# JettHuang/jet-pbrt

Measured on AMD Instinct MI355X. Metric: Msamples/sec (whole node) + per-pixel L2 vs CPU ref, cornell_box 1024spp, higher is better.
Workload: dtype f32

## Files before the change

### jet-pbrt_amd/__init__.py

```python
import ctypes as C
import os

PKG_DIR = os.path.dirname(os.path.abspath(__file__))
REPO_DIR = os.path.dirname(PKG_DIR)
HIP_LIB_PATH = os.environ.get("JETPBRT_AMD_LIB") or os.path.join(PKG_DIR, "csrc", "libjetpbrt_amd.so")
HOST_LIB_PATH = os.path.join(PKG_DIR, "host", "libjetpbrt_host.so")
CLI_PATH = os.path.join(PKG_DIR, "host", "jetpbrt")

JP_MAT_PARAM_STRIDE = 16
JP_SAMPLER_STOCK_MT19937, JP_SAMPLER_COUNTER, JP_SAMPLER_DEBUG = 0, 1, 2
JP_OK = 0

_fp = C.POINTER(C.c_float)
_ip = C.POINTER(C.c_int32)


class JpCamera(C.Structure):
    _fields_ = [("pos", C.c_float * 3), ("front", C.c_float * 3), ("right", C.c_float * 3), ("up", C.c_float * 3),
                ("res_x", C.c_float), ("res_y", C.c_float)]


class JpScene(C.Structure):
    _fields_ = [
        ("camera", JpCamera),
# ... 1060 lines not shown
        return i

    def set_normal_maps(self, maps):
        self._check(self.lib.jp_set_normal_maps(self.h, None if maps is None else C.byref(maps)))

    def normal_map_info(self):
        i = JpNormalMapInfo()
        i.struct_bytes = C.sizeof(JpNormalMapInfo)
        self._check(self.lib.jp_get_normal_map_info(self.h, C.byref(i)))
        return i

    def set_texture_sampling(self, sampling):
        self._check(self.lib.jp_set_texture_sampling(self.h, None if sampling is None else C.byref(sampling)))

    def texture_sampling_info(self):
        i = JpTexSamplingInfo()
        i.struct_bytes = C.sizeof(JpTexSamplingInfo)
        self._check(self.lib.jp_get_texture_sampling_info(self.h, C.byref(i)))
        return i

    def shading_normal(self, origin, direction, tmin, tmax):
        import numpy as np
        n = origin.shape[0]
        o = np.ascontiguousarray(origin, np.float32); d = np.ascontiguousarray(direction, np.float32)
        t0 = np.ascontiguousarray(tmin, np.float32); t1 = np.ascontiguousarray(tmax, np.float32)
        prim = np.zeros(n, np.int32); ng = np.zeros((n, 3), np.float32); ns = np.zeros((n, 3), np.float32)
        p = lambda a: a.ctypes.data_as(C.c_void_p)
        self._check(self.lib.jp_shading_normal(self.h, n, p(o), p(d), p(t0), p(t1), p(prim), p(ng), p(ns)))
        return prim, ng, ns

    def synchronize(self):
        self._check(self.lib.jp_synchronize(self.h))

    def set_profiling(self, on):
        self._check(self.lib.jp_set_profiling(self.h, 1 if on else 0))

    def counters(self):
        c = JpCounters()
        self._check(self.lib.jp_get_counters(self.h, C.byref(c)))
        return c

    def build_info(self):
        b = JpBuildInfo()
        self._check(self.lib.jp_get_build_info(self.h, C.byref(b)))
        return b

    def shadow_kernel(self):
        fn = self.lib.jp_dbg_shadow_kernel
        fn.argtypes = [C.c_void_p, C.POINTER(C.c_int)]; fn.restype = C.c_int
        which = C.c_int(-1)
        self._check(fn(self.h, C.byref(which)))
        return ("refill", "generic", "flat", "pair")[which.value]

    def read_table(self, which):
        return _read_table(lambda out, cap, n: self.lib.jp_read_scene_table(self.h, _table_index(which), out, cap, n))

    def tree_info(self):
        i = JpTreeInfo()
        i.struct_bytes = C.sizeof(JpTreeInfo)
        self._check(self.lib.jp_get_tree_info(self.h, C.byref(i)))
        return i

    def trace(self, origin, direction, tmin, tmax):
        import numpy as np
        n = origin.shape[0]
        o = np.ascontiguousarray(origin, np.float32); d = np.ascontiguousarray(direction, np.float32)
        t0 = np.ascontiguousarray(tmin, np.float32); t1 = np.ascontiguousarray(tmax, np.float32)
        hit = np.zeros(n, np.int32); t = np.zeros(n, np.float32); prim = np.zeros(n, np.int32); nrm = np.zeros((n, 3), np.float32)
        p = lambda a: a.ctypes.data_as(C.c_void_p)
        self._check(self.lib.jp_trace(self.h, n, p(o), p(d), p(t0), p(t1), p(hit), p(t), p(prim), p(nrm)))
        return hit, t, prim, nrm

    def occluded(self, origin, direction, tmin, tmax):
        import numpy as np
        n = origin.shape[0]
        o = np.ascontiguousarray(origin, np.float32); d = np.ascontiguousarray(direction, np.float32)
        t0 = np.ascontiguousarray(tmin, np.float32); t1 = np.ascontiguousarray(tmax, np.float32)
        occ = np.zeros(n, np.int32); walk = C.c_int32(-1)
        p = lambda a: a.ctypes.data_as(C.c_void_p)
        self._check(self.lib.jp_occluded(self.h, n, p(o), p(d), p(t0), p(t1), p(occ), C.byref(walk)))
        return occ, int(walk.value)

    def bsdf(self, desc, normal, wo, wi, u):
        import numpy as np
        n = normal.shape[0]
        a = [np.ascontiguousarray(x, np.float32) for x in (normal, wo, wi, u)]
        out = dict(f=np.zeros((n, 3), np.float32), pdf=np.zeros(n, np.float32), sf=np.zeros((n, 3), np.float32), swi=np.zeros((n, 3), np.float32),
                   spdf=np.zeros(n, np.float32), sflags=np.zeros(n, np.int32))
        p = lambda x: x.ctypes.data_as(C.c_void_p)
        self._check(self.lib.jp_bsdf(self.h, C.byref(desc), n, p(a[0]), p(a[1]), p(a[2]), p(a[3]), p(out["f"]), p(out["pdf"]), p(out["sf"]), p(out["swi"]), p(out["spdf"]), p(out["sflags"])))
        return out

    def close(self):
        if self.h:
            self.lib.jp_destroy_context(self.h)
            self.h = C.c_void_p()

    def __del__(self):
        try:
            self.close()
        except Exception:
            pass


from . import scenes
from . import distributed
# ... 1 lines not shown
```

### jet-pbrt_amd/csrc/jp_device.h

```cpp
#pragma once
#include <hip/hip_runtime.h>
#include <stdint.h>
#include "jetpbrt_amd.h"
#include "jp_counter_rng.h"

#define JP_BLOCK 256
#define JP_STACK_DEPTH 32

namespace jp
{
struct V3 { float x, y, z; };
__device__ __forceinline__ V3 mk(float x, float y, float z) { V3 v; v.x = x; v.y = y; v.z = z; return v; }
__device__ __forceinline__ V3 operator+(V3 a, V3 b) { return mk(a.x + b.x, a.y + b.y, a.z + b.z); }
__device__ __forceinline__ V3 operator-(V3 a, V3 b) { return mk(a.x - b.x, a.y - b.y, a.z - b.z); }
__device__ __forceinline__ V3 operator-(V3 a) { return mk(-a.x, -a.y, -a.z); }
__device__ __forceinline__ V3 operator*(V3 a, float s) { return mk(a.x * s, a.y * s, a.z * s); }
__device__ __forceinline__ V3 operator*(float s, V3 a) { return mk(a.x * s, a.y * s, a.z * s); }
__device__ __forceinline__ V3 operator/(V3 a, float s) { return mk(a.x / s, a.y / s, a.z / s); }
__device__ __forceinline__ V3 cmul(V3 a, V3 b) { return mk(a.x * b.x, a.y * b.y, a.z * b.z); }
__device__ __forceinline__ V3 cdiv(V3 a, V3 b) { return mk(a.x / b.x, a.y / b.y, a.z / b.z); }
__device__ __forceinline__ V3 splat(float v) { return mk(v, v, v); }
__device__ __forceinline__ V3 csqrt(V3 a) { return mk(sqrtf(a.x), sqrtf(a.y), sqrtf(a.z)); }
__device__ __forceinline__ float dot(V3 a, V3 b) { return a.x * b.x + a.y * b.y + a.z * b.z; }
__device__ __forceinline__ float len2(V3 a) { return a.x * a.x + a.y * a.y + a.z * a.z; }
// ... 334 lines not shown
		#pragma unroll
		for (int u = 0; u < 4; u++) JP_FLAT_BOX(i0 + u)
	}
	for (; i0 < n_flat; i0++) JP_FLAT_BOX(i0)
	#undef JP_FLAT_BOX
	#undef JP_FLAT_BOX_RAY
	mA = maskA; mB = maskB;
}

template <int kS, typename PrimPtr>
__device__ __forceinline__ void flat_prims_pair(unsigned int mA, unsigned int mB, PrimPtr prims, V3 o, V3 dA, V3 dB, float tmin, float tmaxA, float tmaxB, bool& hitA, bool& hitB)
{
	bool hA = false, hB = false;
	unsigned int todo = mA | mB;
	while (todo)
	{
		const int p = __ffs((int)todo) - 1;
		const unsigned int bit = todo & (0u - todo);
		todo &= todo - 1;
		const float4 g0 = prims[kS * p + 0], g1 = prims[kS * p + 1], g2 = prims[kS * p + 2], g3 = prims[kS * p + 3];
		const V3 n = xyz(g3);
		const V3 oa = xyz(g0) - o;
		const float noa = dot(n, oa);
		const float distA = noa / dot(n, dA), distB = noa / dot(n, dB);
		const bool passA = (mA & bit) && (distA > tmin) && (distA < tmaxA);
		const bool passB = (mB & bit) && (distB > tmin) && (distB < tmaxB);
		if (passA || passB)
		{
			const V3 ob = xyz(g1) - o, oc = xyz(g2) - o;
			const V3 v0 = cross(oc, ob), v1 = cross(ob, oa);
			const float v0A = dot(v0, dA), v1A = dot(v1, dA), v0B = dot(v0, dB), v1B = dot(v1, dB);
			bool inA, inB;
			if (__float_as_int(g3.w) == JP_SHAPE_TRIANGLE)
			{
				const V3 v2 = cross(oa, oc);
				const float v2A = dot(v2, dA), v2B = dot(v2, dB);
				inA = ((v0A < 0) && (v1A < 0) && (v2A < 0)) || ((v0A >= 0) && (v1A >= 0) && (v2A >= 0));
				inB = ((v0B < 0) && (v1B < 0) && (v2B < 0)) || ((v0B >= 0) && (v1B >= 0) && (v2B >= 0));
			}
			else
			{
				const V3 od = mk(g0.w, g1.w, g2.w) - o;
				const V3 v2 = cross(oa, od), v3 = cross(od, oc);
				const float v2A = dot(v2, dA), v3A = dot(v3, dA), v2B = dot(v2, dB), v3B = dot(v3, dB);
				inA = ((v0A < 0) && (v1A < 0) && (v2A < 0) && (v3A < 0)) || ((v0A >= 0) && (v1A >= 0) && (v2A >= 0) && (v3A >= 0));
				inB = ((v0B < 0) && (v1B < 0) && (v2B < 0) && (v3B < 0)) || ((v0B >= 0) && (v1B >= 0) && (v2B >= 0) && (v3B >= 0));
			}
			if (passA && inA) { hA = true; mA = 0; }
			if (passB && inB) { hB = true; mB = 0; }
			todo &= mA | mB;
		}
	}
	hitA = hA; hitB = hB;
}

template <bool kAnyHit, typename PrimPtr>
__device__ __forceinline__ int traverse_wide(const uint4* __restrict__ wide, PrimPtr prims, V3 o, V3 d, float tmin, float& tmax, unsigned int* stack)
{
	const float ix = 1.0f / d.x, iy = 1.0f / d.y, iz = 1.0f / d.z;
	const unsigned int octinv = 7u - ((d.x < 0 ? 1u : 0u) | (d.y < 0 ? 2u : 0u) | (d.z < 0 ? 4u : 0u));
	unsigned int ngx = 0, ngy = 0x80000000u;
	int hit = -1, sp = 0;
	for (;;)
	{
		unsigned int tgx = 0, tgy = 0;
		if (ngy > 0x00ffffffu)
		{
			const unsigned int bit = 31u - (unsigned int)__clz((int)ngy);
			ngy &= ~(1u << bit);
			if (ngy > 0x00ffffffu) { stack[(2 * sp) * JP_BLOCK] = ngx; stack[(2 * sp + 1) * JP_BLOCK] = ngy; sp++; }
			const unsigned int slot = (bit - 24u) ^ octinv;
			const unsigned int rel = (unsigned int)__popc(ngy & 0xffu & ~(0xffffffffu << slot));
			const unsigned int idx = ngx + rel;
			const uint4 q0 = wide[5 * idx + 0], q1 = wide[5 * idx + 1], q2 = wide[5 * idx + 2], q3 = wide[5 * idx + 3], q4 = wide[5 * idx + 4];
			const float sx = __uint_as_float(((q0.w & 0xffu) ) << 23), sy = __uint_as_float(((q0.w >> 8) & 0xffu) << 23), sz = __uint_as_float(((q0.w >> 16) & 0xffu) << 23);
			const float px = __uint_as_float(q0.x) - o.x, py = __uint_as_float(q0.y) - o.y, pz = __uint_as_float(q0.z) - o.z;
			unsigned int hm = 0;
			#pragma unroll
			for (int i = 0; i < 8; i++)
			{
				const int sh = 8 * (i & 3);
				const unsigned int m = ((i < 4 ? q1.z : q1.w) >> sh) & 0xffu;
				const float lx = (float)(((i < 4 ? q2.x : q2.y) >> sh) & 0xffu), ly = (float)(((i < 4 ? q2.z : q2.w) >> sh) & 0xffu), lz = (float)(((i < 4 ? q3.x : q3.y) >> sh) & 0xffu);
				const float hx = (float)(((i < 4 ? q3.z : q3.w) >> sh) & 0xffu), hy = (float)(((i < 4 ? q4.x : q4.y) >> sh) & 0xffu), hz = (float)(((i < 4 ? q4.z : q4.w) >> sh) & 0xffu);
				const float x0 = fmaf(lx, sx, px) * ix, x1 = fmaf(hx, sx, px) * ix;
				const float y0 = fmaf(ly, sy, py) * iy, y1 = fmaf(hy, sy, py) * iy;
				const float z0 = fmaf(lz, sz, pz) * iz, z1 = fmaf(hz, sz, pz) * iz;
				const float tn = fmaxf(fmaxf(fminf(x0, x1), fminf(y0, y1)), fmaxf(fminf(z0, z1), tmin));
				const float tf = fminf(fminf(fmaxf(x0, x1), fmaxf(y0, y1)), fminf(fmaxf(z0, z1), tmax));
				if (m != 0u && tn <= tf * 1.000002f)
				{
					const bool inner = (m & 0x18u) == 0x18u;
					const unsigned int bits = inner ? 1u : (m >> 5), at = inner ? 24u + ((m & 7u) ^ octinv) : (m & 31u);
					hm |= bits << at;
				}
			}
			ngx = q1.x; ngy = (hm & 0xff000000u) | (q0.w >> 24);
			tgx = q1.y; tgy = hm & 0x00ffffffu;
		}
		while (tgy)
		{
			const int j = __ffs((int)tgy) - 1;
			tgy &= tgy - 1;
			if (prim_hit<4>(prims, (int)tgx + j, o, d, tmin, tmax)) { hit = (int)tgx + j; if (kAnyHit) return hit; }
		}
		if (ngy <= 0x00ffffffu)
// ... 287 lines not shown
```

### jet-pbrt_amd/csrc/jp_kernels.hip

```cpp
#include "jp_common.h"
#include "jp_tex.h"
#include "jp_normals.h"
#include "jp_normal_map.h"
#include "jp_env.h"
#include "jp_mis.h"
#include "jp_lens.h"
#include "jp_xbsdf.h"
#include "jp_film.h"

#include <cstdio>
#include <cstring>
#include <string>
#include <vector>
#include <algorithm>
#include <cmath>
#include <mutex>
#include <thread>
#include <tuple>
#include <functional>
#include <type_traits>
#include "jp_devmem.h"
#include "jp_lbvh.h"
#include "jp_ploc.h"

// ... 113 lines not shown

template <> struct SceneAccess<3>
{
	const float4* prims; unsigned int* stack;
	__device__ __forceinline__ SceneAccess(const SceneView& sc, int) : prims(sc.prims), stack((unsigned int*)s_dyn + threadIdx.x) {}
	template <bool kAnyHit> __device__ __forceinline__ int trace(const SceneView& sc, V3 o, V3 d, float tmin, float& tmax) const
	{ return traverse_wide<kAnyHit>(sc.wide, prims, o, d, tmin, tmax, stack); }
};

template <> struct SceneAccess<4>
{
	WalkStack stack;
	__device__ __forceinline__ SceneAccess(const SceneView&, int depth) { stack.lds = (int*)s_dyn + threadIdx.x; stack.spill = nullptr; stack.cap = depth - 1; stack.stride = 0; }
	template <bool kAnyHit> __device__ __forceinline__ int trace(const SceneView& sc, V3 o, V3 d, float tmin, float& tmax) const
	{ return walk_ray<4, kAnyHit>(sc, o, d, tmin, tmax, stack); }
};

template <> struct SceneAccess<6>
{
	WalkStack stack;
	__device__ __forceinline__ SceneAccess(const SceneView&, int depth) { stack.lds = (int*)s_dyn + threadIdx.x; stack.spill = nullptr; stack.cap = depth - 1; stack.stride = 0; }
	template <bool kAnyHit> __device__ __forceinline__ int trace(const SceneView& sc, V3 o, V3 d, float tmin, float& tmax) const
	{ return walk_ray<6, kAnyHit>(sc, o, d, tmin, tmax, stack); }
};

template <> struct SceneAccess<5>
{
	const float4 *nodes, *prims; int* stack;
	__device__ __forceinline__ SceneAccess(const SceneView& sc, int) : nodes(sc.nodes), prims(sc.prims), stack((int*)s_dyn + threadIdx.x) {}
	template <bool kAnyHit> __device__ __forceinline__ int trace(const SceneView&, V3 o, V3 d, float tmin, float& tmax) const
	{ return traverse_ref<kAnyHit>(nodes, prims, o, d, tmin, tmax, stack); }
};

template <int kMode, typename F = FeatAll>
__global__ void __launch_bounds__(JP_BLOCK) k_extend(SceneView sc, Queues q, int cur, int depth, DevCounters* cnt)
{
	SceneAccess<kMode, F> acc(sc, depth);
	const unsigned int b = blockIdx.x, n = q.blk_q[cur][b], rbase = b * q.R;
	if (b == 0 && threadIdx.x == 0) { cnt->closest += cnt->n_queue[cur]; cnt->n_queue[cur ^ 1] = 0; cnt->n_shadow = 0; }
	unsigned int h = 0;
	float4 ro = make_float4(0, 0, 0, 0), rd = make_float4(0, 0, 1, 0);
	if (threadIdx.x < n) { ro = q.ray_o[cur][rbase + threadIdx.x]; rd = q.ray_d[cur][rbase + threadIdx.x]; }
	for (unsigned int j = threadIdx.x; j < n; j += JP_BLOCK)
	{
		const unsigned int i = rbase + j;
		const float4 co = ro, cd = rd;
		if (j + JP_BLOCK < n) { ro = q.ray_o[cur][i + JP_BLOCK]; rd = q.ray_d[cur][i + JP_BLOCK]; }
		float tmax = JP_INF;
		int hit;
		if constexpr (kMode == 2) hit = acc.trace_unbounded(sc, xyz(co), xyz(cd), 0.001f, tmax);
		else hit = acc.template trace<false>(sc, xyz(co), xyz(cd), 0.001f, tmax);
		q.hit[i] = make_float2(tmax, __int_as_float(hit));
		h += hit >= 0 ? 1u : 0u;
	}
	for (int off = 32; off > 0; off >>= 1) h += __shfl_down(h, off);
	if ((threadIdx.x & 63) == 0 && h) atomicAdd(&cnt->closest_hit, (unsigned long long)h);
}

#ifndef JP_SHADE_TILE
#define JP_SHADE_TILE 8192
#endif
template <bool kSmooth> struct SmoothVars { };
template <> struct SmoothVars<true> { float4 next, rec; V3 Ns; bool on, guard; };
template <bool kSmooth> __device__ __forceinline__ V3 shade_n(const SmoothVars<kSmooth>& sm, V3 N) { if constexpr (kSmooth) return sm.Ns; else return N; }
template <bool kSmooth> __device__ __forceinline__ bool shade_refuses(const SmoothVars<kSmooth>& sm, V3 w, V3 wo, V3 Ng)
{
	if constexpr (kSmooth) return sm.guard && dot(w, Ng) * dot(wo, Ng) <= 0.f; else return false;
}
template <bool kTab, bool kPrims, bool kStage, bool kSort, bool kTex, bool kPick, bool kEnv, bool kMis, typename F = FeatAll, bool kOne = false, bool kSmooth = false>
__device__ __forceinline__ void shade_body(SceneView sc, Queues q, RenderConst rc, int cur, DevCounters* cnt, const TexView& tv, const PickView& pv, const EnvView& ev, const MisView& mv, const NormView& nv = NormView())
{
	static_assert(kPick || !kMis, "k_shade: the light strategy's pdf needs the light table");
	static_assert(kTab || !kPrims, "k_shade: primitive records in LDS only together with the tables");
	static_assert(kPick || !kEnv, "k_shade: the map light is an entry of the light table");
	static_assert(!kSmooth || !kPrims, "k_shade: a shading normal has no entry in the frame table");
	constexpr int kWaves = JP_BLOCK / 64, kMaxSeg = (JP_SHADE_TILE / JP_BLOCK) * kWaves;
	static_assert(JP_SHADE_TILE % JP_BLOCK == 0 && JP_SHADE_TILE <= 65536, "k_shade: tile positions are 16-bit");
	__shared__ unsigned short s_idx[kSort ? JP_SHADE_TILE : 1];
	static_assert(!kOne || (kSort && kPrims && !F::delta && !F::other_lights && !kTex && !kPick && !kMis), "k_shade: the one-sweep partition is the lean sorted instance's");
	__shared__ unsigned char s_key[kSort && !kOne ? JP_SHADE_TILE : 1];
	__shared__ unsigned int s_cnt[kSort && !kOne ? JP_SHADE_CLASSES * kMaxSeg : 1];
	__shared__ unsigned int s_two;
	__shared__ unsigned int s_wsum[kWaves];
	__shared__ unsigned int s_ctr[3];
	const unsigned int lane = threadIdx.x & 63u;
	const int n_tab_l = kPick ? 0 : 2 * sc.n_lights;
	const int n_tab = n_tab_l + 4 * sc.n_mats + (sc.n_mats + 3) / 4, n_tab_all = n_tab + (kPrims ? 8 * sc.n_prims : 0);
	float4* s_lights = s_dyn;
	float4* s_mats = s_lights + n_tab_l;
	int* s_mtype = (int*)(s_mats + 4 * sc.n_mats);
	float4* s_prims = s_dyn + n_tab;
	int4* s_meta = (int4*)(s_prims + 4 * sc.n_prims);
	const float4* s_frames = s_prims + 5 * sc.n_prims;
	float4* s_stage = s_dyn + n_tab_all + threadIdx.x;
	const unsigned int b = blockIdx.x, n = q.blk_q[cur][b];
	const int nxt = cur ^ 1;
#ifdef JP_SHADE_TIMING
	unsigned long long t_acc[10] = { 0, 0, 0, 0, 0, 0, 0, 0, 0, 0 }, t_last = __builtin_amdgcn_s_memtime();
#endif
	if (kTab)
	{
		for (int i = threadIdx.x; i < n_tab_all; i += 2 * JP_BLOCK)
		{
			const bool two = i + JP_BLOCK < n_tab_all;
			const float4 a = sc.shade_tab[i], c2 = two ? sc.shade_tab[i + JP_BLOCK] : a;
			s_dyn[i] = a; if (two) s_dyn[i + JP_BLOCK] = c2;
// ... 974 lines not shown
		s.wi = to_world(fr, s.wi);
		feval[3 * i] = f.x; feval[3 * i + 1] = f.y; feval[3 * i + 2] = f.z; pdfeval[i] = pe;
		sf[3 * i] = s.f.x; sf[3 * i + 1] = s.f.y; sf[3 * i + 2] = s.f.z;
		swi[3 * i] = s.wi.x; swi[3 * i + 1] = s.wi.y; swi[3 * i + 2] = s.wi.z;
		spdf[i] = s.pdf; sflags[i] = s.flags;
	}
}

template <int kMode>
__global__ void __launch_bounds__(JP_BLOCK) k_trace(SceneView sc, int depth, int n, const float* o, const float* d, const float* tmin, const float* tmax_in,
                                                    int* hit, float* t, int* prim, float* nrm)
{
	SceneAccess<kMode> acc(sc, depth);
	for (int i = blockIdx.x * JP_BLOCK + threadIdx.x; i < n; i += gridDim.x * JP_BLOCK)
	{
		const V3 ro = mk(o[3 * i], o[3 * i + 1], o[3 * i + 2]), rd = mk(d[3 * i], d[3 * i + 1], d[3 * i + 2]);
		float tmax = tmax_in[i];
		const int h = acc.template trace<false>(sc, ro, rd, tmin[i], tmax);
		hit[i] = h >= 0; t[i] = tmax; prim[i] = h >= 0 ? sc.meta[h].x : -1;
		V3 N = mk(0, 0, 0);
		if (h >= 0)
		{
			const float4 g3 = sc.prims[4 * h + 3]; const int type = __float_as_int(g3.w);
			const V3 p = ro + tmax * rd;
			if (type == JP_SHAPE_TRIANGLE) N = xyz(g3);
			else if (type == JP_SHAPE_RECTANGLE) N = dot(xyz(g3), rd) <= 0 ? xyz(g3) : -xyz(g3);
			else if (type == JP_SHAPE_DISK) N = xyz(sc.prims[4 * h + 1]);
			else N = normalize(p - xyz(sc.prims[4 * h]));
		}
		nrm[3 * i] = N.x; nrm[3 * i + 1] = N.y; nrm[3 * i + 2] = N.z;
	}
}

__global__ void __launch_bounds__(JP_BLOCK) k_trace_flat(SceneView sc, int depth, int n, const float* o, const float* d, const float* tmin, const float* tmax_in,
                                                         int* hit, float* t, int* prim, float* nrm)
{
	SceneAccess<2, FeatFlat> acc(sc, depth);
	for (int i = blockIdx.x * JP_BLOCK + threadIdx.x; i < n; i += gridDim.x * JP_BLOCK)
	{
		const V3 ro = mk(o[3 * i], o[3 * i + 1], o[3 * i + 2]), rd = mk(d[3 * i], d[3 * i + 1], d[3 * i + 2]);
		float tmax = tmax_in[i];
		const int h = acc.template trace<false>(sc, ro, rd, tmin[i], tmax);
		hit[i] = h >= 0; t[i] = tmax; prim[i] = h >= 0 ? sc.meta[h].x : -1;
		V3 N = mk(0, 0, 0);
		if (h >= 0)
		{
			const float4 g3 = sc.prims[4 * h + 3];
			N = (__float_as_int(g3.w) == JP_SHAPE_TRIANGLE || dot(xyz(g3), rd) <= 0) ? xyz(g3) : -xyz(g3);
		}
		nrm[3 * i] = N.x; nrm[3 * i + 1] = N.y; nrm[3 * i + 2] = N.z;
	}
}

template <int kMode, typename F = FeatAll>
__global__ void __launch_bounds__(JP_BLOCK) k_occluded(SceneView sc, int depth, int n, const float* o, const float* d, const float* tmin, const float* tmax_in, int* occluded)
{
	SceneAccess<kMode, F> acc(sc, depth);
	for (int i = blockIdx.x * JP_BLOCK + threadIdx.x; i < n; i += gridDim.x * JP_BLOCK)
	{
		const V3 ro = mk(o[3 * i], o[3 * i + 1], o[3 * i + 2]), rd = mk(d[3 * i], d[3 * i + 1], d[3 * i + 2]);
		float tmax = tmax_in[i];
		occluded[i] = acc.template trace<true>(sc, ro, rd, tmin[i], tmax) >= 0;
	}
}

__global__ void __launch_bounds__(JP_BLOCK, 8) k_texel(SceneView sc, Queues q, int cur, TexView tv)
{
	const unsigned int b = blockIdx.x, n = q.blk_q[cur][b], rbase = b * q.R;
	for (unsigned int j = threadIdx.x; j < n; j += JP_BLOCK)
	{
		const unsigned int i = rbase + j;
		const float2 h = q.hit[i];
		const int pi = __float_as_int(h.y);
		unsigned int w = 0u;
		if (pi >= 0)
		{
			const int4 meta = sc.meta[pi];
			const int t = meta.y >= 0 ? tv.mat_tex[meta.y] : -1;
			if (t >= 0)
			{
				const float4 ro = q.ray_o[cur][i], rd = q.ray_d[cur][i];
				const V3 p = xyz(ro) + h.x * xyz(rd);
				w = tex_sample(tv, t, tex_uv(sc.prims, tv, pi, meta.x, p), p);
			}
		}
		tv.side[i] = w;
	}
}

template <bool kTab, bool kPrims, bool kStage, bool kSort>
__global__ void __launch_bounds__(JP_BLOCK) k_shade_tex(SceneView sc, Queues q, RenderConst rc, int cur, DevCounters* cnt, TexView tv)
{
	const PickView pv = {}; const EnvView ev = {}; const MisView mv = {};
	shade_body<kTab, kPrims, kStage, kSort, true, false, false, false>(sc, q, rc, cur, cnt, tv, pv, ev, mv);
}

template <int kMode>
__global__ void __launch_bounds__(JP_BLOCK) k_surface(SceneView sc, TexView tv, int depth, int n, const float* o, const float* d, const float* tmin, const float* tmax_in,
                                                      int* prim, float* uv, float* albedo, SampView sm)
{
	SceneAccess<kMode> acc(sc, depth);
	for (int i = blockIdx.x * JP_BLOCK + threadIdx.x; i < n; i += gridDim.x * JP_BLOCK)
	{
		const V3 ro = mk(o[3 * i], o[3 * i + 1], o[3 * i + 2]), rd = mk(d[3 * i], d[3 * i + 1], d[3 * i + 2]);
		float tmax = tmax_in[i];
		const int h = acc.template trace<false>(sc, ro, rd, tmin[i], tmax);
// ... 46 lines not shown
```

### jet-pbrt_amd/csrc/jp_render.h

```cpp
#pragma once
namespace
{
enum { CLS_EXTEND = 0, CLS_SHADE = 1, CLS_SHADOW = 2, CLS_OTHER = 3, CLS_PATH = 4, CLS_NORMAL = 5, CLS_NMAP = 6, CLS_TEXEL = 7 };

int lens_plan_of(const JpContext* c, JpLensPlan& lp)
{
	std::memset(&lp, 0, sizeof(lp));
	if (!c->lens_on) return JP_OK;
	if (jp_lens_make_plan(&c->plan.sv.cam, &c->lens, &lp) != 0) return fail(JP_ERR_INVALID_ARGUMENT, "jp_set_lens: the uploaded camera's right / up vectors have no finite positive length");
	return JP_OK;
}

void free_queues(JpContext* c) { c->qb = QueueBufs(); c->cap = 0; c->planes_alloc = 0; c->blk_alloc = 0; }

int ensure_queues(JpContext* c, unsigned int cap, int planes, unsigned int nblocks)
{
	if (c->cap >= cap && c->planes_alloc >= planes && c->blk_alloc >= nblocks) return JP_OK;
	cap = std::max(cap, c->cap); planes = std::max(planes, c->planes_alloc); nblocks = std::max(nblocks, c->blk_alloc);
	free_queues(c);
	auto alloc = [](DevBuf& b, auto*& p, size_t bytes) { return reserve(b, p, bytes) == hipSuccess; };
	Queues& q = c->q; QueueBufs& qb = c->qb; bool ok = true;
	for (int b = 0; b < 2 && ok; b++) ok = alloc(qb.ray_o[b], q.ray_o[b], (size_t)cap * 16) && alloc(qb.ray_d[b], q.ray_d[b], (size_t)cap * 16) && alloc(qb.beta[b], q.beta[b], (size_t)cap * 16)
	                                       && alloc(qb.blk_q[b], q.blk_q[b], (size_t)nblocks * 4);
	ok = ok && alloc(qb.hit, q.hit, (size_t)cap * 8) && alloc(qb.lacc, q.lacc, (size_t)cap * 16) && alloc(qb.sh_o, q.sh_o, (size_t)cap * 16)
// ... 32 lines not shown
	{
		if (!c->profiling) return;
		if (c->evused + 2 > c->evpool.size()) { size_t old = c->evpool.size(); c->evpool.resize(old + 64); for (size_t i = old; i < c->evpool.size(); i++) hipEventCreate(&c->evpool[i]); }
		a = c->evused; c->evused += 2;
		hipEventRecord(c->evpool[a], c->stream);
	}
	~Stamper() { if (!c->profiling) return; hipEventRecord(c->evpool[a + 1], c->stream); JpContext::Stamp s = { cls, a, a + 1 }; c->stamps.push_back(s); }
};

static void launch_texel(JpContext* c, const ScenePlan& p, int grid, int cur, const TexView& tv)
{
	Stamper t(c, CLS_TEXEL);
	if (p.sm.tex) hipLaunchKernelGGL(k_texel_s, dim3(grid), dim3(JP_BLOCK), 0, c->stream, p.sv, c->q, cur, tv, p.sm);
	else hipLaunchKernelGGL(k_texel, dim3(grid), dim3(JP_BLOCK), 0, c->stream, p.sv, c->q, cur, tv);
}
static void launch_normal(JpContext* c, const ScenePlan& p, int grid, int cur, const NormView& nv);

struct Shard { int band, count, index, local_rows, lane_rows; };
int shard_of(const JpRenderParams* rp, Shard& s, int lane_index = 0, int lane_count = 1, int lane_group = 4)
{
	if (rp->width <= 0 || rp->height <= 0 || rp->spp <= 0 || rp->max_depth < 0 || rp->max_depth > 200) return fail(JP_ERR_INVALID_ARGUMENT, "jp_render: bad width/height/spp/max_depth");
	if (rp->integrator < JP_INTEGRATOR_PATH || rp->integrator > JP_INTEGRATOR_DEBUG_NORMAL) return fail(JP_ERR_INVALID_ARGUMENT, "jp_render: unknown integrator");
	if (rp->integrator == JP_INTEGRATOR_WHITTED && rp->max_depth > JP_WHITTED_MAX_DEPTH) return fail(JP_ERR_UNSUPPORTED, "jp_render: the Whitted integrator supports max_depth <= 16");
	if (rp->sampler_mode != JP_SAMPLER_COUNTER && rp->sampler_mode != JP_SAMPLER_DEBUG) return fail(JP_ERR_UNSUPPORTED, "jp_render: the device path implements the counter sampler only (the sequential mt19937_64 stream is not reproducible in parallel)");
	s.band = rp->band_rows > 0 ? rp->band_rows : 20;
	s.count = rp->shard_count > 1 ? rp->shard_count : 1;
	s.index = s.count > 1 ? rp->shard_index : 0;
	if (s.index < 0 || s.index >= s.count) return fail(JP_ERR_INVALID_ARGUMENT, "jp_render: shard_index out of range");
	const int nbands = (rp->height + s.band - 1) / s.band;
	s.local_rows = 0;
	for (int b = s.index; b < nbands; b += s.count) s.local_rows += std::min(s.band, rp->height - b * s.band);
	s.lane_rows = 0;
	for (int g0 = lane_index * lane_group; g0 < s.local_rows; g0 += lane_count * lane_group) s.lane_rows += std::min(lane_group, s.local_rows - g0);
	return JP_OK;
}

inline bool refill_walks(const ScenePlan& p) { return p.persist && (p.trav_mode == 0 || p.trav_mode == 3 || p.trav_mode == 5); }
inline int refill_row(const ScenePlan& p) { return p.persist >= 32 ? 2 : (p.persist >= 16 ? 1 : 0); }
inline int extend_depth(const ScenePlan& p) { return (p.trav_mode == 5 ? p.cert : p.use_q4) ? p.stack_depth_q4 : p.stack_depth; }
inline int shadow_depth(const ScenePlan& p) { return (p.trav_mode == 5 ? p.cert : p.q4_shadow) ? p.stack_depth_q4 : (p.trav_mode == 3 ? (int)(p.lds_bytes_shadow / (JP_BLOCK * sizeof(int))) : p.stack_depth); }
inline int deepest_walk(const ScenePlan& p) { return std::max(std::max(p.stack_depth, p.stack_depth_q4), p.trav_mode == 3 ? (int)(p.lds_bytes_shadow / (JP_BLOCK * sizeof(int))) : 0); }
inline size_t spill_need(const ScenePlan& p, int deep, unsigned int G) { return deep >= p.stack_lds_words ? (size_t)(deep - p.stack_lds_words + 1) * G * JP_BLOCK : 1; }

inline bool flat_shapes_only(int shape_mask) { return (shape_mask & ~((1 << JP_SHAPE_TRIANGLE) | (1 << JP_SHAPE_RECTANGLE))) == 0; }
inline bool lean_traversal(const ScenePlan& p, bool generic) { return !generic && p.trav_mode == 2 && flat_shapes_only(p.shape_mask); }
inline bool lean_shading(const ScenePlan& p, bool generic)
{
	const int delta_classes = (2 << JP_MAT_MIRROR) | (2 << JP_MAT_GLASS) | (2 << JP_MAT_PLASTIC);
	return !generic && p.shade_prims_in_lds && p.stage_nee && flat_shapes_only(p.shape_mask) && (p.light_mask & ~(1 << JP_LIGHT_AREA)) == 0
	    && flat_shapes_only(p.light_shape_mask) && (p.class_mask & delta_classes) == 0;
}

typedef void (*ExtendKernel)(SceneView, Queues, int, int, DevCounters*);
typedef void (*ExtendRefillKernel)(SceneView, Queues, int, int, int*, DevCounters*);
struct ExtendLaunch { ExtendRefillKernel refill; ExtendKernel plain; size_t lds; int words; };
template <int M> ExtendRefillKernel extend_refill(const ScenePlan& p)
{
	static const ExtendRefillKernel k[3][2] = { { k_extend_persist<M, 8, false>, k_extend_persist<M, 8, true> }, { k_extend_persist<M, 16, false>, k_extend_persist<M, 16, true> }, { k_extend_persist<M, 32, false>, k_extend_persist<M, 32, true> } };
	return k[refill_row(p)][p.vote];
}
ExtendLaunch extend_kernel(const ScenePlan& p, bool generic)
{
	if (lean_traversal(p, generic)) return { nullptr, k_extend<2, FeatFlat>, p.lds_bytes, p.stack_depth };
	if (!refill_walks(p)) return { nullptr, p.trav_mode == 5 ? k_extend<5> : (p.trav_mode == 2 ? k_extend<2> : (p.trav_mode == 1 ? k_extend<1> : k_extend<0>)), p.lds_bytes, p.stack_depth };
	const int words = std::min(extend_depth(p), p.stack_lds_words);
	const ExtendRefillKernel k = p.trav_mode == 5 ? (p.cert ? extend_refill<6>(p) : extend_refill<5>(p)) : (p.use_q4 ? extend_refill<4>(p) : extend_refill<0>(p));
	return { k, nullptr, (size_t)words * JP_BLOCK * sizeof(int), words };
}

typedef void (*ShadowKernel)(SceneView, Queues, RenderConst, int, DevCounters*);
typedef void (*ShadowRefillKernel)(SceneView, Queues, RenderConst, int, int*, DevCounters*);
struct ShadowLaunch { ShadowRefillKernel refill; ShadowKernel plain; size_t lds; int words; bool cert_fell_back; };
template <int M> ShadowRefillKernel shadow_refill(const ScenePlan& p)
{
	static const ShadowRefillKernel k[3][2] = { { k_shadow_persist<M, 8, false>, k_shadow_persist<M, 8, true> }, { k_shadow_persist<M, 16, false>, k_shadow_persist<M, 16, true> }, { k_shadow_persist<M, 32, false>, k_shadow_persist<M, 32, true> } };
	return k[refill_row(p)][p.vote];
}
ShadowLaunch shadow_kernel(const ScenePlan& p, unsigned int R, bool generic)
{
	const int words = std::min(shadow_depth(p), p.stack_lds_words);
	const size_t plds = (size_t)words * JP_BLOCK * sizeof(int) + (((size_t)R * p.n_planes + 31) / 32) * 4 * (p.cert ? 2 : 1);
#ifndef JP_NO_SHADOW_PAIR
	if (lean_traversal(p, generic) && p.sv.n_prims <= 32 && p.n_planes >= 2) return { nullptr, k_shadow_pair, p.lds_bytes, p.stack_depth, p.cert };
#endif
	if (lean_traversal(p, generic)) return { nullptr, k_shadow<2, FeatFlat>, p.lds_bytes, p.stack_depth, p.cert };
	if (!refill_walks(p) || plds > 64 * 1024)
		return { nullptr, p.trav_mode == 3 ? k_shadow<3> : (p.trav_mode == 5 ? k_shadow<5> : (p.trav_mode == 2 ? k_shadow<2> : (p.trav_mode == 1 ? k_shadow<1> : k_shadow<0>))), p.trav_mode == 3 ? p.lds_bytes_shadow : p.lds_bytes, p.stack_depth, p.cert };
	const ShadowRefillKernel k = p.trav_mode == 5 ? (p.cert ? shadow_refill<6>(p) : shadow_refill<5>(p)) : (p.q4_shadow ? shadow_refill<4>(p) : (p.trav_mode == 3 ? shadow_refill<3>(p) : shadow_refill<0>(p)));
	return { k, nullptr, plds, words, false };
}

enum { SHADE_PLAIN = 0, SHADE_LEAN, SHADE_LEAN_ONE, SHADE_PICK, SHADE_ENV, SHADE_MIS, SHADE_MIS_ENV };
enum { ROW_TTT = 0, ROW_TTF, ROW_TFT, ROW_TFF, ROW_FFF };
struct ShadeChoice { int family; bool tex, smooth; int row; bool sort; };
ShadeChoice shade_choice(const ScenePlan& p, bool tex, bool mis, bool smooth, bool generic)
{
	ShadeChoice c;
	c.family = mis ? (p.env ? SHADE_MIS_ENV : SHADE_MIS) : (p.env ? SHADE_ENV : (p.pick ? SHADE_PICK : SHADE_PLAIN));
	c.tex = tex; c.smooth = smooth; c.sort = p.shade_sort;
	c.row = p.shade_prims_in_lds ? (p.stage_nee ? ROW_TTT : ROW_TTF) : (p.tables_in_lds ? (p.stage_nee ? ROW_TFT : ROW_TFF) : ROW_FFF);
	if (c.family == SHADE_PLAIN && !tex && !smooth && lean_shading(p, generic))
	{
		c.family = SHADE_LEAN;
#ifndef JP_NO_ONE_SWEEP
		if (p.shade_sort && !p.has_null_material) c.family = SHADE_LEAN_ONE;
#endif
	}
	return c;
}
typedef std::tuple<TexView, PickView, EnvView, MisView, NormView> ShadeViews;
typedef std::function<void(hipStream_t, int, size_t, const SceneView&, const Queues&, const RenderConst&, int, DevCounters*)> ShadeLaunch;
ShadeLaunch shade_launch(const ShadeChoice& c, const ShadeViews& views);
}
static int film_to_rgb8(JpContext* c, const float* src, int width, int height);
static int ensure_mis_side(JpContext* c, unsigned int cap, MisView& mv);
static int ensure_normal_side(JpContext* c, unsigned int cap, NormView& nv);
namespace
{

typedef void (*OtherKernel)(SceneView, Queues, RenderConst, int, int, DevCounters*, int, JpLensPlan);
OtherKernel other_kernel(const ScenePlan& p) { return p.trav_mode == 5 ? k_other<5> : (p.trav_mode == 2 ? k_other<2> : (p.trav_mode == 1 ? k_other<1> : k_other<0>)); }

typedef void (*TraceKernel)(SceneView, int, int, const float*, const float*, const float*, const float*, int*, float*, int*, float*);
typedef void (*SurfaceKernel)(SceneView, TexView, int, int, const float*, const float*, const float*, const float*, int*, float*, float*, SampView);
struct TraceLaunch { TraceKernel trace; SurfaceKernel surface; size_t lds; int depth; int mode; };
template <int M> TraceLaunch trace_row(size_t lds, int depth) { TraceLaunch t = { k_trace<M>, k_surface<M>, lds, depth, M }; return t; }
template <class F> auto by_trace_mode(int mode, F f) -> decltype(f(std::integral_constant<int, 0>()))
{
	switch (mode)
	{
	case 0: return f(std::integral_constant<int, 0>());
	case 1: return f(std::integral_constant<int, 1>());
	case 2: return f(std::integral_constant<int, 2>());
	case 4: return f(std::integral_constant<int, 4>());
	case 5: return f(std::integral_constant<int, 5>());
	case 6: return f(std::integral_constant<int, 6>());
	default: return nullptr;
	}
}
TraceLaunch trace_kernel(const ScenePlan& p, int tw, bool generic = true)
{
	const size_t q4lds = (size_t)p.stack_depth_q4 * JP_BLOCK * sizeof(int);
	if (p.trav_mode == 3 && tw == 2) { TraceLaunch t = { k_trace<3>, nullptr, p.lds_bytes_shadow, p.stack_depth, 3 }; return t; }
	if (p.trav_mode == 5 && p.cert && q4lds <= 64 * 1024 && tw != 3) return trace_row<6>(q4lds, p.stack_depth_q4);
	if (p.trav_mode == 5) return trace_row<5>(p.lds_bytes, p.stack_depth);
	if (p.use_q4 && q4lds <= 64 * 1024 && tw != 1) return trace_row<4>(q4lds, p.stack_depth_q4);
	if (lean_traversal(p, generic)) { TraceLaunch t = { k_trace_flat, k_surface<2>, p.lds_bytes, p.stack_depth, 2 + 16 }; return t; }
	return p.trav_mode == 2 ? trace_row<2>(p.lds_bytes, p.stack_depth) : (p.trav_mode == 1 ? trace_row<1>(p.lds_bytes, p.stack_depth) : trace_row<0>(p.lds_bytes, p.stack_depth));
}

typedef void (*OccludedKernel)(SceneView, int, int, const float*, const float*, const float*, const float*, int*);
struct OccludedLaunch { OccludedKernel occluded; size_t lds; int depth; int walk; };
template <int M> OccludedLaunch occluded_row(size_t lds, int depth) { OccludedLaunch t = { k_occluded<M>, lds, depth, M }; return t; }
OccludedLaunch occluded_kernel(const ScenePlan& p, int tw, bool generic)
{
	const size_t q4lds = (size_t)p.stack_depth_q4 * JP_BLOCK * sizeof(int);
	if (p.trav_mode == 3 && tw == 2) return occluded_row<3>(p.lds_bytes_shadow, p.stack_depth);
	if (p.trav_mode == 5 && p.cert && q4lds <= 64 * 1024 && tw != 3) return occluded_row<6>(q4lds, p.stack_depth_q4);
	if (p.trav_mode == 5) return occluded_row<5>(p.lds_bytes, p.stack_depth);
	if (p.q4_shadow && q4lds <= 64 * 1024 && tw != 1) return occluded_row<4>(q4lds, p.stack_depth_q4);
	if (p.trav_mode == 3 && tw != 1) return occluded_row<3>(p.lds_bytes_shadow, p.stack_depth);
	if (lean_traversal(p, generic)) { OccludedLaunch t = { k_occluded<2, FeatFlat>, p.lds_bytes, p.stack_depth, 2 + 16 }; return t; }
	return p.trav_mode == 2 ? occluded_row<2>(p.lds_bytes, p.stack_depth) : (p.trav_mode == 1 ? occluded_row<1>(p.lds_bytes, p.stack_depth) : occluded_row<0>(p.lds_bytes, p.stack_depth));
}

int render_one(JpContext* c, const JpRenderParams* rp, float* film_dev, bool sync, int lane_index = 0, int lane_count = 1, int lane_group = 4, bool ev0_recorded = false)
{
	if (!c->plan.have_scene) return fail(JP_ERR_NO_SCENE, "jp_render: no scene uploaded");
	const ScenePlan& p = c->plan; Shard sh; DevCounters* const d_cnt = c->cnt.get<DevCounters>();
	if (const int e = shard_of(rp, sh, lane_index, lane_count, lane_group); e != JP_OK) return e;
	HIP_TRY(hipSetDevice(c->device));
	const long long npix = (long long)sh.lane_rows * rp->width;

	if (!ev0_recorded) HIP_TRY(hipEventRecord(c->ev0, c->stream));
	HIP_TRY(hipMemsetAsync(film_dev, 0, sizeof(float) * 3 * (size_t)rp->width * rp->height, c->stream));
	HIP_TRY(hipMemsetAsync(d_cnt, 0, sizeof(DevCounters), c->stream));
	c->evused = 0; c->stamps.clear();
	unsigned long long samples = 0;
	if (npix > 0)
	{
		if (npix > (1 << 24)) return fail(JP_ERR_UNSUPPORTED, "jp_render: more than 2^24 pixels per shard");
		const int slot_bits = p.n_planes <= 31 ? 27 : 24;
		const unsigned int PMAX = slot_bits == 27 ? (1u << 26) : (1u << 24);
		size_t freeB = 0, totalB = 0; hipMemGetInfo(&freeB, &totalB);
		const bool smooth = p.smooth && rp->integrator == JP_INTEGRATOR_PATH;
		const size_t per = 136 + 32 * (size_t)p.n_planes + (smooth ? 16 : 0);
		size_t budget = std::min<size_t>((size_t)24 << 30, (freeB / (size_t)std::max(1, lane_count) + (c->cap ? (size_t)c->cap * (136 + 32 * (size_t)c->planes_alloc) : 0)) / 2);
		if (c->opt.max_slots > 0) budget = std::min<size_t>(budget, (size_t)c->opt.max_slots * per);
		int sbatch = 1; unsigned int P = 0, G = 1, R = JP_BLOCK, cap = 0;
		for (int attempt = 0;; attempt++)
		{
			const unsigned int pcap = (unsigned int)std::min<size_t>(PMAX, std::max<size_t>((size_t)npix, budget / per));
			sbatch = (int)std::max<long long>(1, std::min<long long>(rp->spp, pcap / npix));
			{
				const int nb = (rp->spp + sbatch - 1) / sbatch;
				sbatch = (rp->spp + nb - 1) / nb;
			}
			if ((long long)sbatch * npix > (long long)PMAX) return fail(JP_ERR_UNSUPPORTED, "jp_render: shard too large for one batch");
			P = (unsigned int)((long long)sbatch * npix);
// ... 486 lines not shown
	HIP_TRY(hipMemcpyAsync(d_t0, tmin, (size_t)n * 4, hipMemcpyHostToDevice, c->stream)); HIP_TRY(hipMemcpyAsync(d_t1, tmax, (size_t)n * 4, hipMemcpyHostToDevice, c->stream));
	const int grid = std::min(c->n_cus * 8, (n + JP_BLOCK - 1) / JP_BLOCK);
	hipLaunchKernelGGL(ok.occluded, dim3(grid), dim3(JP_BLOCK), ok.lds, c->stream, c->plan.sv, ok.depth, n, d_o, d_d, d_t0, d_t1, d_occ);
	HIP_TRY(hipGetLastError());
	HIP_TRY(hipMemcpyAsync(occluded, d_occ, (size_t)n * 4, hipMemcpyDeviceToHost, c->stream));
	HIP_TRY(hipStreamSynchronize(c->stream));
	return JP_OK;
}

int jp_get_texture_info(JpContext* c, JpTextureInfo* out)
{
	if (!c || !out) return fail(JP_ERR_INVALID_ARGUMENT, "jp_get_texture_info: null argument");
	if (out->struct_bytes < (int32_t)sizeof(int32_t)) return fail(JP_ERR_INVALID_ARGUMENT, "jp_get_texture_info: set JpTextureInfo.struct_bytes to sizeof(JpTextureInfo)");
	JpTextureInfo i; std::memset(&i, 0, sizeof(i));
	i.n_textures = c->plan.textured ? c->n_textures : 0; i.n_textured_materials = c->n_tex_mats; i.texel_bytes_device = c->texel_bytes; i.textured_last_render = c->last_textured;
	const size_t n = std::min((size_t)out->struct_bytes, sizeof(i));
	i.struct_bytes = (int32_t)n;
	std::memcpy(out, &i, n);
	return JP_OK;
}

int jp_surface(JpContext* c, int32_t n, const float* origin, const float* dir, const float* tmin, const float* tmax, int32_t* prim, float* uv, float* albedo)
{
	if (!c || n < 0 || !origin || !dir || !tmin || !tmax || !prim || !uv || !albedo) return fail(JP_ERR_INVALID_ARGUMENT, "jp_surface: null argument");
	if (!c->plan.have_scene) return fail(JP_ERR_NO_SCENE, "jp_surface: no scene uploaded");
	if (n == 0) return JP_OK;
	HIP_TRY(hipSetDevice(c->device));
	DevBuf b_in, b_uv, b_a, b_prim; float *d_in, *d_uv, *d_a; int* d_prim;
	HIP_TRY(reserve(b_in, d_in, (size_t)n * 32)); HIP_TRY(reserve(b_uv, d_uv, (size_t)n * 8)); HIP_TRY(reserve(b_a, d_a, (size_t)n * 12)); HIP_TRY(reserve(b_prim, d_prim, (size_t)n * 4));
	float *d_o = d_in, *d_d = d_in + 3 * (size_t)n, *d_t0 = d_in + 6 * (size_t)n, *d_t1 = d_in + 7 * (size_t)n;
	HIP_TRY(hipMemcpyAsync(d_o, origin, (size_t)n * 12, hipMemcpyHostToDevice, c->stream)); HIP_TRY(hipMemcpyAsync(d_d, dir, (size_t)n * 12, hipMemcpyHostToDevice, c->stream));
	HIP_TRY(hipMemcpyAsync(d_t0, tmin, (size_t)n * 4, hipMemcpyHostToDevice, c->stream)); HIP_TRY(hipMemcpyAsync(d_t1, tmax, (size_t)n * 4, hipMemcpyHostToDevice, c->stream));
	const int grid = std::min(c->n_cus * 8, (n + JP_BLOCK - 1) / JP_BLOCK);
	const TraceLaunch tk = trace_kernel(c->plan, 0);
	hipLaunchKernelGGL(tk.surface, dim3(grid), dim3(JP_BLOCK), tk.lds, c->stream, c->plan.sv, c->plan.tv, tk.depth, n, d_o, d_d, d_t0, d_t1, d_prim, d_uv, d_a, c->plan.sm);
	HIP_TRY(hipGetLastError());
	HIP_TRY(hipMemcpyAsync(prim, d_prim, (size_t)n * 4, hipMemcpyDeviceToHost, c->stream)); HIP_TRY(hipMemcpyAsync(uv, d_uv, (size_t)n * 8, hipMemcpyDeviceToHost, c->stream));
	HIP_TRY(hipMemcpyAsync(albedo, d_a, (size_t)n * 12, hipMemcpyDeviceToHost, c->stream));
	HIP_TRY(hipStreamSynchronize(c->stream));
	return JP_OK;
}

}

extern "C" int jp_dbg_shadow_kernel(JpContext* c, int* which_out)
{
	if (!c || !which_out) return fail(JP_ERR_INVALID_ARGUMENT, "jp_dbg_shadow_kernel: null argument");
	if (!c->plan.have_scene) return fail(JP_ERR_NO_SCENE, "jp_dbg_shadow_kernel: no scene uploaded");
	const ShadowLaunch sk = shadow_kernel(c->plan, c->q.R ? c->q.R : JP_BLOCK, c->opt.reserved[0] == 1);
	*which_out = sk.refill ? 0 : (sk.plain == (ShadowKernel)k_shadow_pair ? 3 : (sk.plain == (ShadowKernel)k_shadow<2, FeatFlat> ? 2 : 1));
	return JP_OK;
}

#if defined(JP_SHADE_TIMING) || defined(JP_TRAV_TIMING)
extern "C" int jp_dbg_shade_timing(unsigned long long* out16)
{
	unsigned long long z[16] = { 0 };
	if (hipMemcpyFromSymbol(out16, HIP_SYMBOL(g_shade_t), sizeof(z)) != hipSuccess) return -1;
	if (hipMemcpyToSymbol(HIP_SYMBOL(g_shade_t), z, sizeof(z)) != hipSuccess) return -1;
	return 0;
}
#endif

#ifdef JP_WALK_STATS
extern "C" int jp_dbg_walk_stats(unsigned long long* out8)
{
	unsigned long long z[8] = { 0 };
	if (hipMemcpyFromSymbol(out8, HIP_SYMBOL(jp::g_walk_stats), sizeof(z)) != hipSuccess) return -1;
	if (hipMemcpyToSymbol(HIP_SYMBOL(jp::g_walk_stats), z, sizeof(z)) != hipSuccess) return -1;
	return 0;
}
extern "C" int jp_dbg_turn_stats(unsigned long long* out32)
{
	unsigned long long z[32] = { 0 };
	if (hipMemcpyFromSymbol(out32, HIP_SYMBOL(jp::g_turn_stats), sizeof(z)) != hipSuccess) return -1;
	if (hipMemcpyToSymbol(HIP_SYMBOL(jp::g_turn_stats), z, sizeof(z)) != hipSuccess) return -1;
	return 0;
}
#endif

#ifdef JP_PATH_TIMING
extern "C" int jp_dbg_path_timing(unsigned long long* out16)
{
	unsigned long long z[16] = { 0 };
	if (hipMemcpyFromSymbol(out16, HIP_SYMBOL(g_path_t), sizeof(z)) != hipSuccess) return -1;
	if (hipMemcpyToSymbol(HIP_SYMBOL(g_path_t), z, sizeof(z)) != hipSuccess) return -1;
	return 0;
}
#endif
```

Baseline: 3411.

## Add wave-pooled primitive testing for flat scenes with few primitives

Adds extend and trace kernels for flat-BVH scenes with at most 32 primitives. Each wave pushes its (ray, primitive) candidate pairs from the box test into an LDS ring, then intersects them 64 at a time across all lanes. Each ray's nearest hit is kept with a wave-scope atomic min on a packed (t, prim) slot. The aim is to remove the divergence of lanes looping over different numbers of candidate primitives, at the cost of extra LDS use, fences and atomics.

```diff
diff --git a/jet-pbrt_amd/__init__.py b/jet-pbrt_amd/__init__.py
--- a/jet-pbrt_amd/__init__.py
+++ b/jet-pbrt_amd/__init__.py
@@ -1136,6 +1136,13 @@
         self._check(fn(self.h, C.byref(which)))
         return ("refill", "generic", "flat", "pair")[which.value]
 
+    def extend_kernel(self):
+        fn = self.lib.jp_dbg_extend_kernel
+        fn.argtypes = [C.c_void_p, C.POINTER(C.c_int)]; fn.restype = C.c_int
+        which = C.c_int(-1)
+        self._check(fn(self.h, C.byref(which)))
+        return ("refill", "generic", "flat", "pool")[which.value]
+
     def read_table(self, which):
         return _read_table(lambda out, cap, n: self.lib.jp_read_scene_table(self.h, _table_index(which), out, cap, n))
 
diff --git a/jet-pbrt_amd/csrc/jp_device.h b/jet-pbrt_amd/csrc/jp_device.h
--- a/jet-pbrt_amd/csrc/jp_device.h
+++ b/jet-pbrt_amd/csrc/jp_device.h
@@ -410,6 +410,50 @@
 		}
 	}
 	hitA = hA; hitB = hB;
+}
+
+#define JP_POOL_RING 128
+#define JP_POOL_WAVE_BYTES (64 * 32 + 64 * 8 + JP_POOL_RING * 2)
+template <bool kUniform, int kS, typename PrimPtr>
+__device__ __forceinline__ void pool_round(PrimPtr prims, const float4* rays, u64* slots, const unsigned short* ring, unsigned int head, unsigned int n_valid,
+                                           unsigned int lane, float tmin_u, float tmax_u)
+{
+	if (lane < n_valid)
+	{
+		const unsigned int e = ring[(head + lane) & (JP_POOL_RING - 1)];
+		const unsigned int owner = e >> 8, p = e & 0xffu;
+		const float4 r0 = rays[2 * owner], r1 = rays[2 * owner + 1];
+		float t = kUniform ? tmax_u : r1.w;
+		if (prim_hit<kS, FeatFlat>(prims, (int)p, xyz(r0), mk(r0.w, r1.x, r1.y), kUniform ? tmin_u : r1.z, t))
+			__hip_atomic_fetch_min(&slots[owner], ((u64)__float_as_uint(t) << 32) | (u64)p, __ATOMIC_RELAXED, __HIP_MEMORY_SCOPE_WAVEFRONT);
+	}
+}
+
+template <bool kUniform, int kS, typename PrimPtr>
+__device__ __forceinline__ int flat_prims_pool(unsigned int mask, PrimPtr prims, V3 o, V3 d, float tmin, float& tmax, float4* rays, u64* slots, unsigned short* ring)
+{
+	const unsigned int lane = __builtin_amdgcn_mbcnt_hi(~0u, __builtin_amdgcn_mbcnt_lo(~0u, 0u));
+	rays[2 * lane] = make_float4(o.x, o.y, o.z, d.x); rays[2 * lane + 1] = make_float4(d.y, d.z, tmin, tmax);
+	slots[lane] = ~(u64)0;
+	__builtin_amdgcn_fence(__ATOMIC_RELEASE, "wavefront");
+	unsigned int head = 0, tail = 0;
+	for (u64 live = __ballot(mask != 0); live; live = __ballot(mask != 0))
+	{
+		const unsigned int rank = __builtin_amdgcn_mbcnt_hi((unsigned int)(live >> 32), __builtin_amdgcn_mbcnt_lo((unsigned int)live, 0u));
+		const unsigned int entry = (lane << 8) | (unsigned int)(__ffs((int)mask) - 1);
+		if (mask) ring[(tail + rank) & (JP_POOL_RING - 1)] = (unsigned short)entry;
+		mask &= mask - 1;
+		tail += (unsigned int)__popcll(live);
+		__builtin_amdgcn_fence(__ATOMIC_ACQ_REL, "wavefront");
+		if (tail - head >= 64u) { pool_round<kUniform, kS>(prims, rays, slots, ring, head, 64u, lane, tmin, tmax); head += 64u; }
+	}
+	if (tail != head) pool_round<kUniform, kS>(prims, rays, slots, ring, head, tail - head, lane, tmin, tmax);
+	__builtin_amdgcn_fence(__ATOMIC_ACQ_REL, "wavefront");
+	const u64 best = slots[lane];
+	__builtin_amdgcn_fence(__ATOMIC_ACQUIRE, "wavefront");
+	if (best == ~(u64)0) return -1;
+	tmax = __uint_as_float((unsigned int)(best >> 32));
+	return (int)(unsigned int)best;
 }
 
 template <bool kAnyHit, typename PrimPtr>
diff --git a/jet-pbrt_amd/csrc/jp_kernels.hip b/jet-pbrt_amd/csrc/jp_kernels.hip
--- a/jet-pbrt_amd/csrc/jp_kernels.hip
+++ b/jet-pbrt_amd/csrc/jp_kernels.hip
@@ -189,6 +189,39 @@
 		else hit = acc.template trace<false>(sc, xyz(co), xyz(cd), 0.001f, tmax);
 		q.hit[i] = make_float2(tmax, __int_as_float(hit));
 		h += hit >= 0 ? 1u : 0u;
+	}
+	for (int off = 32; off > 0; off >>= 1) h += __shfl_down(h, off);
+	if ((threadIdx.x & 63) == 0 && h) atomicAdd(&cnt->closest_hit, (unsigned long long)h);
+}
+
+struct PoolLds
+{
+	float4* rays; u64* slots; unsigned short* ring;
+	__device__ __forceinline__ PoolLds(int n_prims)
+	{
+		char* base = (char*)(s_dyn + 5 * n_prims) + (threadIdx.x >> 6) * JP_POOL_WAVE_BYTES;
+		rays = (float4*)base; slots = (u64*)(base + 64 * 32); ring = (unsigned short*)(base + 64 * 32 + 64 * 8);
+	}
+};
+
+__global__ void __launch_bounds__(JP_BLOCK, 8) k_extend_pool(SceneView sc, Queues q, int cur, int depth, DevCounters* cnt)
+{
+	SceneAccess<2, FeatFlat> acc(sc, depth);
+	const PoolLds pool(sc.n_prims);
+	const unsigned int b = blockIdx.x, n = q.blk_q[cur][b], rbase = b * q.R;
+	if (b == 0 && threadIdx.x == 0) { cnt->closest += cnt->n_queue[cur]; cnt->n_queue[cur ^ 1] = 0; cnt->n_shadow = 0; }
+	unsigned int h = 0;
+	float4 ro = make_float4(0, 0, 0, 0), rd = make_float4(0, 0, 1, 0);
+	if (threadIdx.x < n) { ro = q.ray_o[cur][rbase + threadIdx.x]; rd = q.ray_d[cur][rbase + threadIdx.x]; }
+	for (unsigned int j0 = threadIdx.x & ~63u; j0 < n; j0 += JP_BLOCK)
+	{
+		const unsigned int j = j0 + (threadIdx.x & 63u), i = rbase + j;
+		const float4 co = ro, cd = rd;
+		if (j + JP_BLOCK < n) { ro = q.ray_o[cur][i + JP_BLOCK]; rd = q.ray_d[cur][i + JP_BLOCK]; }
+		float tmax = JP_INF;
+		const unsigned int m = flat_boxes_lean<true>(sc.flat, sc.n_flat, xyz(co), xyz(cd), 0.001f, tmax);
+		const int hit = flat_prims_pool<true, 5>(j < n ? m : 0u, acc.prims, xyz(co), xyz(cd), 0.001f, tmax, pool.rays, pool.slots, pool.ring);
+		if (j < n) { q.hit[i] = make_float2(tmax, __int_as_float(hit)); h += hit >= 0 ? 1u : 0u; }
 	}
 	for (int off = 32; off > 0; off >>= 1) h += __shfl_down(h, off);
 	if ((threadIdx.x & 63) == 0 && h) atomicAdd(&cnt->closest_hit, (unsigned long long)h);
@@ -1269,6 +1302,35 @@
 	}
 }
 
+__global__ void __launch_bounds__(JP_BLOCK, 8) k_trace_pool(SceneView sc, int depth, int n, const float* o, const float* d, const float* tmin, const float* tmax_in,
+                                                            int* hit, float* t, int* prim, float* nrm)
+{
+	SceneAccess<2, FeatFlat> acc(sc, depth);
+	const PoolLds pool(sc.n_prims);
+	for (int i0 = blockIdx.x * JP_BLOCK + (threadIdx.x & ~63); i0 < n; i0 += gridDim.x * JP_BLOCK)
+	{
+		const int i = i0 + (threadIdx.x & 63);
+		const bool live = i < n;
+		V3 ro = mk(0, 0, 0), rd = mk(0, 0, 1); float t0 = 0.001f, tmax = JP_INF;
+		if (live) { ro = mk(o[3 * i], o[3 * i + 1], o[3 * i + 2]); rd = mk(d[3 * i], d[3 * i + 1], d[3 * i + 2]); t0 = tmin[i]; tmax = tmax_in[i]; }
+		const unsigned int m0 = flat_boxes_lean<false>(sc.flat, sc.n_flat, ro, rd, t0, tmax), m = live ? m0 : 0u;
+		int h;
+		if (__ballot(!(t0 >= 0.f)) == 0) h = flat_prims_pool<false, 5>(m, acc.prims, ro, rd, t0, tmax, pool.rays, pool.slots, pool.ring);
+		else h = flat_prims<false, false, 5, FeatFlat>(m, acc.prims, ro, rd, t0, tmax);
+		if (live)
+		{
+			hit[i] = h >= 0; t[i] = tmax; prim[i] = h >= 0 ? sc.meta[h].x : -1;
+			V3 N = mk(0, 0, 0);
+			if (h >= 0)
+			{
+				const float4 g3 = sc.prims[4 * h + 3];
+				N = (__float_as_int(g3.w) == JP_SHAPE_TRIANGLE || dot(xyz(g3), rd) <= 0) ? xyz(g3) : -xyz(g3);
+			}
+			nrm[3 * i] = N.x; nrm[3 * i + 1] = N.y; nrm[3 * i + 2] = N.z;
+		}
+	}
+}
+
 template <int kMode, typename F = FeatAll>
 __global__ void __launch_bounds__(JP_BLOCK) k_occluded(SceneView sc, int depth, int n, const float* o, const float* d, const float* tmin, const float* tmax_in, int* occluded)
 {
diff --git a/jet-pbrt_amd/csrc/jp_render.h b/jet-pbrt_amd/csrc/jp_render.h
--- a/jet-pbrt_amd/csrc/jp_render.h
+++ b/jet-pbrt_amd/csrc/jp_render.h
@@ -108,6 +108,7 @@
 }
 
 typedef void (*ExtendKernel)(SceneView, Queues, int, int, DevCounters*);
+inline size_t pool_lds_bytes() { return (size_t)(JP_BLOCK / 64) * JP_POOL_WAVE_BYTES; }
 typedef void (*ExtendRefillKernel)(SceneView, Queues, int, int, int*, DevCounters*);
 struct ExtendLaunch { ExtendRefillKernel refill; ExtendKernel plain; size_t lds; int words; };
 template <int M> ExtendRefillKernel extend_refill(const ScenePlan& p)
@@ -117,6 +118,9 @@
 }
 ExtendLaunch extend_kernel(const ScenePlan& p, bool generic)
 {
+#ifndef JP_NO_EXTEND_POOL
+	if (lean_traversal(p, generic) && p.sv.n_prims <= 32) return { nullptr, k_extend_pool, p.lds_bytes + pool_lds_bytes(), p.stack_depth };
+#endif
 	if (lean_traversal(p, generic)) return { nullptr, k_extend<2, FeatFlat>, p.lds_bytes, p.stack_depth };
 	if (!refill_walks(p)) return { nullptr, p.trav_mode == 5 ? k_extend<5> : (p.trav_mode == 2 ? k_extend<2> : (p.trav_mode == 1 ? k_extend<1> : k_extend<0>)), p.lds_bytes, p.stack_depth };
 	const int words = std::min(extend_depth(p), p.stack_lds_words);
@@ -201,6 +205,9 @@
 	if (p.trav_mode == 5 && p.cert && q4lds <= 64 * 1024 && tw != 3) return trace_row<6>(q4lds, p.stack_depth_q4);
 	if (p.trav_mode == 5) return trace_row<5>(p.lds_bytes, p.stack_depth);
 	if (p.use_q4 && q4lds <= 64 * 1024 && tw != 1) return trace_row<4>(q4lds, p.stack_depth_q4);
+#ifndef JP_NO_EXTEND_POOL
+	if (lean_traversal(p, generic) && p.sv.n_prims <= 32) { TraceLaunch t = { k_trace_pool, k_surface<2>, p.lds_bytes + pool_lds_bytes(), p.stack_depth, 2 + 16 }; return t; }
+#endif
 	if (lean_traversal(p, generic)) { TraceLaunch t = { k_trace_flat, k_surface<2>, p.lds_bytes, p.stack_depth, 2 + 16 }; return t; }
 	return p.trav_mode == 2 ? trace_row<2>(p.lds_bytes, p.stack_depth) : (p.trav_mode == 1 ? trace_row<1>(p.lds_bytes, p.stack_depth) : trace_row<0>(p.lds_bytes, p.stack_depth));
 }
@@ -793,6 +800,15 @@
 	return JP_OK;
 }
 
+extern "C" int jp_dbg_extend_kernel(JpContext* c, int* which_out)
+{
+	if (!c || !which_out) return fail(JP_ERR_INVALID_ARGUMENT, "jp_dbg_extend_kernel: null argument");
+	if (!c->plan.have_scene) return fail(JP_ERR_NO_SCENE, "jp_dbg_extend_kernel: no scene uploaded");
+	const ExtendLaunch ek = extend_kernel(c->plan, c->opt.reserved[0] == 1);
+	*which_out = ek.refill ? 0 : (ek.plain == (ExtendKernel)k_extend_pool ? 3 : (ek.plain == (ExtendKernel)k_extend<2, FeatFlat> ? 2 : 1));
+	return JP_OK;
+}
+
 #if defined(JP_SHADE_TIMING) || defined(JP_TRAV_TIMING)
 extern "C" int jp_dbg_shade_timing(unsigned long long* out16)
 {
```

After: 3522 (median of 6 runs). 3.2% higher.
